# jgsimard/big-dreamer

Measured on AMD Instinct MI355X. Metric: latent transitions/sec (RSSM + imagination) at batch=50 chunk=50 H=15, higher is better.
Workload: dtype f32

## Files before the change

### big_dreamer_amd/csrc/wgrad.hip

```cpp
#include "bd_device.h"
#include "bd_host.h"
#include <stdint.h>
#include <stdlib.h>

namespace bd {

typedef float floatx16 __attribute__((ext_vector_type(16)));
constexpr int kWT = 64;
constexpr int kWM = 32;

__global__ __launch_bounds__(kThreads) void wgrad_kernel(const float* __restrict__ dpre, int ldp,
                                                         const float* __restrict__ act, int lda, int M, int N, int K,
                                                         int has_bias, int rows_per_split, float* __restrict__ ws) {
    __shared__ float P[kWM][kWT];
    __shared__ float A[kWM][kWT];
    const int Kext = K + has_bias;
    const int n0 = blockIdx.x * kWT, k0 = blockIdx.y * kWT;
    const int m_begin = blockIdx.z * rows_per_split;
    const int m_end = min(M, m_begin + rows_per_split);
    const int lane = threadIdx.x & 63, wave = threadIdx.x >> 6;
    const int wn = (wave >> 1) * 32, wk = (wave & 1) * 32;
    floatx16 acc;
#pragma unroll
    for (int i = 0; i < 16; ++i) acc[i] = 0.f;
    const int c = threadIdx.x & 63, r0 = threadIdx.x >> 6;
    for (int m0 = m_begin; m0 < m_end; m0 += kWM) {
        float pv[kWM / 4], av[kWM / 4];
#pragma unroll
        for (int i = 0; i < kWM / 4; ++i) {
            const int m = m0 + r0 + 4 * i;
            const bool ok = m < m_end;
            pv[i] = (ok && n0 + c < N) ? dpre[(size_t)m * ldp + n0 + c] : 0.f;
            const int k = k0 + c;
            av[i] = ok ? (k < K ? act[(size_t)m * lda + k] : (k == K && has_bias ? 1.f : 0.f)) : 0.f;
        }
        __syncthreads();
#pragma unroll
        for (int i = 0; i < kWM / 4; ++i) {
            P[r0 + 4 * i][c] = pv[i];
            A[r0 + 4 * i][c] = av[i];
        }
        __syncthreads();
#pragma unroll
        for (int s = 0; s < kWM / 2; ++s) {
            const float a = P[2 * s + (lane >> 5)][wn + (lane & 31)];
            const float b = A[2 * s + (lane >> 5)][wk + (lane & 31)];
            acc = __builtin_amdgcn_mfma_f32_32x32x2f32(a, b, acc, 0, 0, 0);
        }
    }
    float* slab = ws + (size_t)blockIdx.z * N * Kext;
    const int k = k0 + wk + (lane & 31);
#pragma unroll
    for (int reg = 0; reg < 16; ++reg) {
        const int n = n0 + wn + (reg & 3) + 8 * (reg >> 2) + 4 * (lane >> 5);
        if (n < N && k < Kext) slab[(size_t)n * Kext + k] = acc[reg];
    }
}

__global__ __launch_bounds__(256) void wgrad_reduce_kernel(const float* __restrict__ ws, int splits, int N, int K,
                                                           int has_bias, float* __restrict__ dW, int ldw,
                                                           float* __restrict__ db, int accumulate) {
    const int Kext = K + has_bias;
    const int total = N * Kext;
    for (int e = blockIdx.x * blockDim.x + threadIdx.x; e < total; e += gridDim.x * blockDim.x) {
        float s = 0.f;
        for (int z = 0; z < splits; ++z) s += ws[(size_t)z * total + e];
        const int n = e / Kext, k = e - n * Kext;
        float* dst = k < K ? dW + (size_t)n * ldw + k : db + n;
        *dst = accumulate ? *dst + s : s;
    }
}

__global__ __launch_bounds__(kThreads) void wgrad_grouped_kernel(const bd_wgrad_desc* __restrict__ descs, int n,
                                                                 float* __restrict__ ws) {
    __shared__ float P[kWM][kWT];
    __shared__ float A[kWM][kWT];
    int g = 0;
    while (g + 1 < n && (int)blockIdx.x >= descs[g + 1].block_begin) ++g;
    const bd_wgrad_desc d = descs[g];
    const int hb = d.db != nullptr;
    const int Kext = d.K + hb;
    int local = blockIdx.x - d.block_begin;
    const int z = local / (d.tiles_n * d.tiles_k);
    local -= z * d.tiles_n * d.tiles_k;
    const int n0 = (local / d.tiles_k) * kWT, k0 = (local % d.tiles_k) * kWT;
    const int m_begin = z * d.rows_per;
    const int m_end = min(d.M, m_begin + d.rows_per);
    const int lane = threadIdx.x & 63, wave = threadIdx.x >> 6;
    const int wn = (wave >> 1) * 32, wk = (wave & 1) * 32;
    floatx16 acc;
#pragma unroll
    for (int i = 0; i < 16; ++i) acc[i] = 0.f;
    const int c = threadIdx.x & 63, r0 = threadIdx.x >> 6;
    float pv[kWM / 4], av[kWM / 4];
    auto fetch = [&](int m0) {
#pragma unroll
        for (int i = 0; i < kWM / 4; ++i) {
            const int m = m0 + r0 + 4 * i;
            const bool ok = m < m_end;
            pv[i] = (ok && n0 + c < d.N) ? d.dpre[(size_t)m * d.ldp + n0 + c] : 0.f;
            const int k = k0 + c;
            float v = 0.f;
            if (ok) {
                if (k < d.K) v = m < d.M1 ? d.act1[(size_t)m * d.lda1 + k] : d.act2[(size_t)(m - d.M1) * d.lda2 + k];
                else if (k == d.K && hb) v = 1.f;
            }
            av[i] = v;
        }
    };
    fetch(m_begin);
    for (int m0 = m_begin; m0 < m_end; m0 += kWM) {
        __syncthreads();
#pragma unroll
        for (int i = 0; i < kWM / 4; ++i) {
            P[r0 + 4 * i][c] = pv[i];
            A[r0 + 4 * i][c] = av[i];
        }
        __syncthreads();
        if (m0 + kWM < m_end) fetch(m0 + kWM);
#pragma unroll
        for (int s = 0; s < kWM / 2; ++s) {
            const float a = P[2 * s + (lane >> 5)][wn + (lane & 31)];
            const float b = A[2 * s + (lane >> 5)][wk + (lane & 31)];
            acc = __builtin_amdgcn_mfma_f32_32x32x2f32(a, b, acc, 0, 0, 0);
        }
    }
    float* slab = ws + d.ws_off + (size_t)z * d.N * Kext;
    const int k = k0 + wk + (lane & 31);
#pragma unroll
    for (int reg = 0; reg < 16; ++reg) {
        const int nn = n0 + wn + (reg & 3) + 8 * (reg >> 2) + 4 * (lane >> 5);
        if (nn < d.N && k < Kext) slab[(size_t)nn * Kext + k] = acc[reg];
    }
}

constexpr int kWB = 13;
constexpr int kWBK = 12;
constexpr int kWBKDeep = 36;
__host__ __device__ __forceinline__ int wgrad_tiles_k(int NB, int KB, bool deep_ok) {
    if (KB <= kWB) return 1;
    return (NB <= 4 && deep_ok) ? cdiv(KB, kWBKDeep) : cdiv(KB, kWBK);
}
__host__ inline bool wgrad_act16(const bd_wgrad_desc& d) {
    auto al16 = [](const void* q) { return (reinterpret_cast<uintptr_t>(q) & 15) == 0; };
    if ((d.K & 3) != 0 || !al16(d.act1)) return false;
    if (d.g_nseg > 0) return (d.g_C & 3) == 0 && (d.g_seglen & 3) == 0;
    return (d.lda1 & 3) == 0 && (d.M1 == d.M || ((d.lda2 & 3) == 0 && al16(d.act2)));
}
constexpr int kWLd = 240;
constexpr int kWRows = 16;
constexpr int kWStage = 2 * kWRows * kWLd;
constexpr int kWRing = 3;
constexpr int kWRowsTall = 32;
constexpr int kWLdNarrow = 80;
constexpr int kWLdMid = 144;
constexpr int kWLdDeep = 592;
constexpr size_t kWideLdsBytes = 147456;
static_assert((size_t)kWRing * kWRows * (kWLdNarrow + kWLdDeep) * sizeof(float) <= kWideLdsBytes, "deep stage ring");
static_assert((size_t)kWRing * kWRowsTall * (kWLdMid + kWLd) * sizeof(float) <= kWideLdsBytes, "mid stage ring");
constexpr int kWThreads = 512;

template <int WN, int WK, int ROWS = kWRows, int PLD = kWLd, int ALD = kWLd>
__device__ __forceinline__ void wgrad_wide_body(const bd_wgrad_desc& d, float* __restrict__ ws, float* wlds, int hb, int Kext,
                                                int z, int n0, int k0, int nb_cnt, int kb_cnt) {
    const int m_begin = z * d.rows_per;
    const int m_end = min(d.M, m_begin + d.rows_per);
    const int lane = threadIdx.x & 63;
    const int wave = __builtin_amdgcn_readfirstlane(threadIdx.x >> 6);
    const int wr = wave & 1, wc = wave >> 1;
    const int hn = (nb_cnt + 1) >> 1;
    const int my_nb0 = wr ? hn : 0, my_nb = wr ? nb_cnt - hn : hn;
    const int kq = kb_cnt >> 2, krem = kb_cnt & 3;
    const int my_kb0 = wc * kq + min(wc, krem), my_kb = kq + (wc < krem ? 1 : 0);

    constexpr int kStage = ROWS * (PLD + ALD);
    constexpr int kRpw = ROWS / 8;
    static_assert(kWRing * kStage * sizeof(float) <= kWideLdsBytes, "stage ring exceeds the LDS request");
    floatx4 acc[WN][WK];
#pragma unroll
    for (int i = 0; i < WN; ++i)
#pragma unroll
        for (int j = 0; j < WK; ++j) acc[i][j] = floatx4{0.f, 0.f, 0.f, 0.f};

    typedef __attribute__((address_space(3))) void* lds_ptr_t;
    typedef const __attribute__((address_space(1))) void* glb_ptr_t;
    const int ncol = min(nb_cnt * 16, d.N - n0), kcol = min(kb_cnt * 16, d.K - k0);
    for (int i = threadIdx.x; i < kWRing * kStage; i += kWThreads) wlds[i] = 0.f;
    __syncthreads();
    if (hb && d.K >= k0 && d.K < k0 + kb_cnt * 16 && threadIdx.x < kWRing * ROWS)
        wlds[(threadIdx.x / ROWS) * kStage + ROWS * PLD + (threadIdx.x % ROWS) * ALD + (d.K - k0)] = 1.f;
    auto al16 = [](const void* q) { return (reinterpret_cast<uintptr_t>(q) & 15) == 0; };
    const bool p4 = (ncol & 3) == 0 && (d.ldp & 3) == 0 && al16(d.dpre + n0);
    const bool gathered = d.g_nseg > 0;
    const bool a4 = (kcol & 3) == 0 && (k0 & 3) == 0 &&
                    (gathered ? ((d.g_C & 3) == 0 && (d.g_seglen & 3) == 0 && al16(d.act1))
                              : ((d.lda1 & 3) == 0 && al16(d.act1) && (d.M1 == d.M || ((d.lda2 & 3) == 0 && al16(d.act2)))));
    constexpr int kCh4 = (ALD + 255) / 256;
    constexpr int kCh1 = (ALD + 63) / 64;
    constexpr int kGo = kCh1;
    int goff[kGo];
#pragma unroll
    for (int cc = 0; cc < kGo; ++cc) goff[cc] = 0;
    if (gathered) {
#pragma unroll
        for (int cc = 0; cc < kGo; ++cc) {
            const int k = k0 + (a4 ? 4 * lane + 256 * cc : lane + 64 * cc), sgm = k / d.g_seglen;
            goff[cc] = sgm * d.g_IW * d.g_C + (k - sgm * d.g_seglen);
        }
    }
    auto issue = [&](float* buf, int m0) {
#pragma unroll
        for (int rr = 0; rr < kRpw; ++rr) {
            const int m = m0 + wave * kRpw + rr;
            float* P = buf + (wave * kRpw + rr) * PLD;
            float* A = buf + ROWS * PLD + (wave * kRpw + rr) * ALD;
            if (m < m_end) {
                const float* prow = d.dpre + (size_t)m * d.ldp + n0;
                if (p4) {
                    if (4 * lane < ncol) __builtin_amdgcn_global_load_lds((glb_ptr_t)(prow + 4 * lane), (lds_ptr_t)P, 16, 0, 0);
                } else {
#pragma unroll
                    for (int cc = 0; cc < 4; ++cc) {
                        const int c = lane + 64 * cc;
                        if (c < ncol) __builtin_amdgcn_global_load_lds((glb_ptr_t)(prow + c), (lds_ptr_t)(P + 64 * cc), 4, 0, 0);
                    }
                }
                const float* abase;
                if (gathered) {
                    const int img = m / (d.g_gh * d.g_gw), rem = m - img * d.g_gh * d.g_gw;
                    const int y = rem / d.g_gw, x = rem - y * d.g_gw;
                    abase = d.act1 + (((size_t)img * d.g_IH + 2 * y) * d.g_IW + 2 * x) * d.g_C;
                } else {
                    abase = (m < d.M1 ? d.act1 + (size_t)m * d.lda1 : d.act2 + (size_t)(m - d.M1) * d.lda2) + k0;
                }
                if (a4) {
#pragma unroll
                    for (int cc = 0; cc < kCh4; ++cc)
                        if (4 * lane + 256 * cc < kcol)
                            __builtin_amdgcn_global_load_lds((glb_ptr_t)(abase + (gathered ? goff[cc] : 4 * lane + 256 * cc)),
                                                             (lds_ptr_t)(A + 256 * cc), 16, 0, 0);
                } else {
#pragma unroll
                    for (int cc = 0; cc < kCh1; ++cc) {
                        const int c = lane + 64 * cc;
                        if (c < kcol)
                            __builtin_amdgcn_global_load_lds((glb_ptr_t)(abase + (gathered ? goff[cc] : c)), (lds_ptr_t)(A + 64 * cc), 4,
                                                             0, 0);
                    }
                }
            } else {
#pragma unroll
                for (int cc = 0; cc < kCh1; ++cc) {
                    const int c = lane + 64 * cc;
                    if (c < PLD) P[c] = 0.f;
                    if (c < ALD) A[c] = 0.f;
                }
            }
        }
    };
    const int nst = cdiv(m_end - m_begin, ROWS);
    const int n_dma = kRpw * ((p4 ? 1 : cdiv(ncol, 64)) + (a4 ? cdiv(kcol, 256) : cdiv(kcol, 64)));
    auto wait_keep_newest = [&]() {
        switch (n_dma) {
            case 4: asm volatile("s_waitcnt vmcnt(4)" ::: "memory"); break;
            case 6: asm volatile("s_waitcnt vmcnt(6)" ::: "memory"); break;
            case 8: asm volatile("s_waitcnt vmcnt(8)" ::: "memory"); break;
            case 10: asm volatile("s_waitcnt vmcnt(10)" ::: "memory"); break;
            case 12: asm volatile("s_waitcnt vmcnt(12)" ::: "memory"); break;
            case 14: asm volatile("s_waitcnt vmcnt(14)" ::: "memory"); break;
            default: asm volatile("s_waitcnt vmcnt(16)" ::: "memory"); break;
        }
    };
    __syncthreads();
    issue(wlds, m_begin);
    if (nst > 1) issue(wlds + kStage, m_begin + ROWS);
    __builtin_amdgcn_s_waitcnt(0);
    __syncthreads();
    const int lrow = lane >> 4, lcol = lane & 15;
    for (int st = 0; st < nst; ++st) {
        const float* buf = wlds + (st % kWRing) * kStage;
        const bool more = st + 2 < nst;
        [[maybe_unused]] const int sb = (st == 10 || st == 11) ? (st - 10) * 8 : -1;
        BD_DSTAMP(sb, 0);
        if (more) issue(wlds + ((st + 2) % kWRing) * kStage, m_begin + (st + 2) * ROWS);
        BD_DSTAMP(sb, 1);
        const float* Pb = buf + lrow * PLD + my_nb0 * 16 + lcol;
        const float* Ab = buf + ROWS * PLD + lrow * ALD + my_kb0 * 16 + lcol;
#pragma unroll
        for (int sl = 0; sl < ROWS / 4; ++sl) {
            float a[WN], b[WK];
#pragma unroll
            for (int i = 0; i < WN; ++i) a[i] = Pb[sl * 4 * PLD + i * 16];
#pragma unroll
            for (int j = 0; j < WK; ++j) b[j] = Ab[sl * 4 * ALD + j * 16];
#pragma unroll
            for (int i = 0; i < WN; ++i)
#pragma unroll
                for (int j = 0; j < WK; ++j) acc[i][j] = mfma16(a[i], b[j], acc[i][j]);
        }
        BD_DSTAMP(sb, 2);
        if (more && st + 3 < nst) wait_keep_newest();
        else asm volatile("s_waitcnt vmcnt(0)" ::: "memory");
        BD_DSTAMP(sb, 3);
        lds_barrier();
        BD_DSTAMP(sb, 4);
    }
    float* slab = ws + d.ws_off + (size_t)z * d.N * Kext;
#pragma unroll
    for (int i = 0; i < WN; ++i) {
        if (i < my_nb) {
#pragma unroll
            for (int j = 0; j < WK; ++j) {
                if (j < my_kb) {
                    const int k = k0 + (my_kb0 + j) * 16 + lcol;
#pragma unroll
                    for (int r = 0; r < 4; ++r) {
                        const int nn = n0 + (my_nb0 + i) * 16 + 4 * lrow + r;
                        if (nn < d.N && k < Kext) slab[(size_t)nn * Kext + k] = acc[i][j][r];
                    }
                }
            }
        }
    }
}

template <int WN, int WK>
__device__ __forceinline__ void wgrad_dense_body(const bd_wgrad_desc& d, float* __restrict__ ws, float* wlds, int hb, int Kext,
                                                 int z, int n0, int k0, int nb_cnt, int kb_cnt, int my_nb0, int my_kb0) {
    const int m_begin = z * d.rows_per;
    const int m_end = min(d.M, m_begin + d.rows_per);
    const int lane = threadIdx.x & 63;
    const int wave = __builtin_amdgcn_readfirstlane(threadIdx.x >> 6);
    floatx4 acc[WN][WK];
#pragma unroll
    for (int i = 0; i < WN; ++i)
#pragma unroll
        for (int j = 0; j < WK; ++j) acc[i][j] = floatx4{0.f, 0.f, 0.f, 0.f};
    typedef __attribute__((address_space(3))) void* lds_ptr_t;
    typedef const __attribute__((address_space(1))) void* glb_ptr_t;
    const int ncol = min(nb_cnt * 16, d.N - n0), kcol = min(kb_cnt * 16, d.K - k0);
    for (int i = threadIdx.x; i < kWRing * kWStage; i += kWThreads) wlds[i] = 0.f;
    __syncthreads();
    if (hb && d.K >= k0 && d.K < k0 + kb_cnt * 16 && threadIdx.x < kWRing * kWRows)
        wlds[(threadIdx.x >> 4) * kWStage + kWRows * kWLd + (threadIdx.x & 15) * kWLd + (d.K - k0)] = 1.f;
    const bool lp = 4 * lane < ncol, la = 4 * lane < kcol;
    const float* __restrict__ pl = d.dpre + n0 + 4 * lane;
    const float* __restrict__ a1l = d.act1 + k0 + 4 * lane;
    const float* __restrict__ a2l = (d.M1 < d.M ? d.act2 : d.act1) + k0 + 4 * lane;
    auto issue = [&](float* buf, int m0) {
#pragma unroll
        for (int rr = 0; rr < 2; ++rr) {
            const int m = m0 + wave * 2 + rr;
            float* P = buf + (wave * 2 + rr) * kWLd;
            float* A = P + kWRows * kWLd;
            if (m < m_end) {
                if (lp) __builtin_amdgcn_global_load_lds((glb_ptr_t)(pl + (size_t)m * d.ldp), (lds_ptr_t)P, 16, 0, 0);
                const float* ar = m < d.M1 ? a1l + (size_t)m * d.lda1 : a2l + (size_t)(m - d.M1) * d.lda2;
                if (la) __builtin_amdgcn_global_load_lds((glb_ptr_t)ar, (lds_ptr_t)A, 16, 0, 0);
            } else {
#pragma unroll
                for (int cc = 0; cc < 4; ++cc) {
                    const int c = lane + 64 * cc;
                    if (c < kWLd) {
                        P[c] = 0.f;
                        A[c] = 0.f;
                    }
                }
            }
        }
    };
    const int nst = cdiv(m_end - m_begin, kWRows);
    __syncthreads();
    issue(wlds, m_begin);
    if (nst > 1) issue(wlds + kWStage, m_begin + kWRows);
    __builtin_amdgcn_s_waitcnt(0);
    __syncthreads();
    const int lrow = lane >> 4, lcol = lane & 15;
    for (int st = 0; st < nst; ++st) {
        const float* buf = wlds + (st % kWRing) * kWStage;
        const bool more = st + 2 < nst;
        [[maybe_unused]] const int sb = (st == 10 || st == 11) ? (st - 10) * 8 : -1;
        BD_DSTAMP(sb, 0);
        if (more && wave < 4) issue(wlds + ((st + 2) % kWRing) * kWStage, m_begin + (st + 2) * kWRows);
        BD_DSTAMP(sb, 1);
        const float* Pb = buf + lrow * kWLd + my_nb0 * 16 + lcol;
        const float* Ab = buf + kWRows * kWLd + lrow * kWLd + my_kb0 * 16 + lcol;
#pragma unroll
        for (int sl = 0; sl < kWRows / 4; ++sl) {
            float a[WN], b[WK];
#pragma unroll
            for (int i = 0; i < WN; ++i) a[i] = Pb[sl * 4 * kWLd + i * 16];
#pragma unroll
            for (int j = 0; j < WK; ++j) b[j] = Ab[sl * 4 * kWLd + j * 16];
#pragma unroll
            for (int i = 0; i < WN; ++i)
#pragma unroll
                for (int j = 0; j < WK; ++j) acc[i][j] = mfma16(a[i], b[j], acc[i][j]);
            if (sl == 1 && more && wave >= 4) issue(wlds + ((st + 2) % kWRing) * kWStage, m_begin + (st + 2) * kWRows);
        }
        BD_DSTAMP(sb, 2);
        if (more && st + 3 < nst) asm volatile("s_waitcnt vmcnt(4)" ::: "memory");
        else asm volatile("s_waitcnt vmcnt(0)" ::: "memory");
        BD_DSTAMP(sb, 3);
        lds_barrier();
        BD_DSTAMP(sb, 4);
    }
    float* slab = ws + d.ws_off + (size_t)z * d.N * Kext;
#pragma unroll
    for (int i = 0; i < WN; ++i) {
#pragma unroll
        for (int j = 0; j < WK; ++j) {
            const int k = k0 + (my_kb0 + j) * 16 + lcol;
#pragma unroll
            for (int r = 0; r < 4; ++r) {
                const int nn = n0 + (my_nb0 + i) * 16 + 4 * lrow + r;
                if (nn < d.N && k < Kext) slab[(size_t)nn * Kext + k] = acc[i][j][r];
            }
        }
    }
}

constexpr int kThinMaxKB = 7;
constexpr int kThinDpreFloats = 1024;
__host__ __device__ inline int thin_band_floats(int k, int roww) { return (k * roww + 64 + 255) & ~255; }
__host__ inline bool wgrad_thin_ok(const bd_wgrad_desc& d) {
    auto al16 = [](const void* q) { return (reinterpret_cast<uintptr_t>(q) & 15) == 0; };
    if (d.g_nseg <= 0 || d.g_C > 4 || d.N != 32 || d.ldp != 32 || d.g_gw > 32) return false;
    if (cdiv(d.K, 16) > kThinMaxKB || d.g_seglen != d.g_nseg * d.g_C) return false;
    const int roww = d.g_IW * d.g_C;
    if ((roww & 3) != 0 || !al16(d.act1) || !al16(d.dpre)) return false;
    const size_t per_wave = 2 * (size_t)(thin_band_floats(d.g_nseg, roww) + kThinDpreFloats) * sizeof(float);
    return 8 * per_wave <= kWideLdsBytes && (size_t)8 * 2 * kThinMaxKB * 1024 <= kWideLdsBytes;
}

#ifndef BD_WGRAD_TALL_MID
#define BD_WGRAD_TALL_MID 1
#endif
__device__ __forceinline__ bool tall_mid() { return BD_WGRAD_TALL_MID != 0; }

template <int KB>
__device__ __forceinline__ void wgrad_thin_body(const bd_wgrad_desc& d, float* __restrict__ ws, float* wlds, int z) {
    typedef __attribute__((address_space(3))) void* lds_ptr_t;
    typedef const __attribute__((address_space(1))) void* glb_ptr_t;
    const int lane = threadIdx.x & 63;
    const int wave = __builtin_amdgcn_readfirstlane(threadIdx.x >> 6);
    const int hb = d.db != nullptr;
    const int Kext = d.K + hb;
    const int gh = d.g_gh, gw = d.g_gw, C = d.g_C, kk = d.g_nseg;
    const int roww = d.g_IW * C, band = kk * roww, drow = gw * 32;
    const int band_al = thin_band_floats(kk, roww);
    const int per_buf = band_al + kThinDpreFloats;
    float* mine = wlds + (size_t)wave * 2 * per_buf;
    for (int i = lane; i < 2 * per_buf; i += 64) mine[i] = 0.f;
    asm volatile("s_waitcnt lgkmcnt(0)" ::: "memory");
    const int imgs = d.M / (gh * gw), ipw = d.rows_per / (gh * gw);
    const int img0 = z * ipw, img1 = min(imgs, img0 + ipw);
    const int items = (img1 - img0) * gh;
    const int nband = cdiv(band, 256), ndrow = cdiv(drow, 256);
    auto issue = [&](int it, float* buf) {
        const int img = img0 + it / gh, y = it - (it / gh) * gh;
        const float* sb = d.act1 + ((size_t)img * d.g_IH + 2 * y) * roww;
        const float* sd = d.dpre + ((size_t)img * gh + y) * gw * 32;
        for (int ch = 0; ch < nband; ++ch)
            if (4 * lane + 256 * ch < band)
                __builtin_amdgcn_global_load_lds((glb_ptr_t)(sb + 4 * lane + 256 * ch), (lds_ptr_t)(buf + 256 * ch), 16, 0, 0);
        for (int ch = 0; ch < ndrow; ++ch)
            if (4 * lane + 256 * ch < drow)
                __builtin_amdgcn_global_load_lds((glb_ptr_t)(sd + 4 * lane + 256 * ch), (lds_ptr_t)(buf + band_al + 256 * ch), 16, 0, 0);
    };
    const int n_dma = nband + ndrow;
    auto wait_keep_newest = [&]() {
        switch (n_dma) {
            case 5: asm volatile("s_waitcnt vmcnt(5)" ::: "memory"); break;
            case 6: asm volatile("s_waitcnt vmcnt(6)" ::: "memory"); break;
            case 7: asm volatile("s_waitcnt vmcnt(7)" ::: "memory"); break;
            case 8: asm volatile("s_waitcnt vmcnt(8)" ::: "memory"); break;
            case 9: asm volatile("s_waitcnt vmcnt(9)" ::: "memory"); break;
            case 10: asm volatile("s_waitcnt vmcnt(10)" ::: "memory"); break;
            default: asm volatile("s_waitcnt vmcnt(0)" ::: "memory"); break;
        }
    };
    int boff[KB];
    bool bok[KB];
#pragma unroll
    for (int kb = 0; kb < KB; ++kb) {
        const int kidx = kb * 16 + (lane & 15);
        bok[kb] = kidx < d.K;
        const int ky = kidx / d.g_seglen;
        boff[kb] = bok[kb] ? ky * roww + (kidx - ky * d.g_seglen) : 0;
    }
    floatx4 acc[2][KB];
#pragma unroll
    for (int i = 0; i < 2; ++i)
#pragma unroll
        for (int j = 0; j < KB; ++j) acc[i][j] = floatx4{0.f, 0.f, 0.f, 0.f};
    float bsum[2] = {0.f, 0.f};
    const int q = lane >> 4, n = lane & 15;
    const int nsl = cdiv(gw, 4);
    int it = wave, b = 0;
    if (it < items) issue(it, mine);
    for (; it < items; it += 8, b ^= 1) {
        const bool more = it + 8 < items;
        if (more) {
            issue(it + 8, mine + (b ^ 1) * per_buf);
            wait_keep_newest();
        } else {
            asm volatile("s_waitcnt vmcnt(0)" ::: "memory");
        }
        const float* Bd = mine + b * per_buf;
        const float* Dp = Bd + band_al;
        for (int sl = 0; sl < nsl; ++sl) {
            const int x = 4 * sl + q;
            const float a0 = Dp[x * 32 + n], a1 = Dp[x * 32 + 16 + n];
            float bv[KB];
#pragma unroll
            for (int kb = 0; kb < KB; ++kb) bv[kb] = bok[kb] ? Bd[boff[kb] + 2 * x * C] : 0.f;
#pragma unroll
            for (int kb = 0; kb < KB; ++kb) {
                acc[0][kb] = mfma16(a0, bv[kb], acc[0][kb]);
                acc[1][kb] = mfma16(a1, bv[kb], acc[1][kb]);
            }
            bsum[0] += a0;
            bsum[1] += a1;
        }
        asm volatile("s_waitcnt lgkmcnt(0)" ::: "memory");
    }
    __syncthreads();
    floatx4* R4 = reinterpret_cast<floatx4*>(wlds);
    float* BS = wlds + (size_t)8 * 2 * KB * 256;
#pragma unroll
    for (int i = 0; i < 2; ++i) {
#pragma unroll
        for (int j = 0; j < KB; ++j) R4[((wave * 2 + i) * KB + j) * 64 + lane] = acc[i][j];
        BS[(wave * 2 + i) * 64 + lane] = bsum[i];
    }
    __syncthreads();
    float* slab = ws + d.ws_off + (size_t)z * d.N * Kext;
    for (int e = threadIdx.x; e < 2 * KB * 64; e += blockDim.x) {
        const int blk = e >> 6, l = e & 63;
        floatx4 s4 = floatx4{0.f, 0.f, 0.f, 0.f};
        for (int w = 0; w < 8; ++w) s4 += R4[(w * 2 * KB + blk) * 64 + l];
        const int i = blk / KB, j = blk - i * KB;
        const int k = j * 16 + (l & 15);
        if (k < d.K) {
#pragma unroll
            for (int r = 0; r < 4; ++r) slab[(size_t)(i * 16 + 4 * (l >> 4) + r) * Kext + k] = s4[r];
        }
    }
    if (hb && threadIdx.x < 32) {
        const int i = threadIdx.x >> 4, nn = threadIdx.x & 15;
        float t = 0.f;
        for (int w = 0; w < 8; ++w)
            for (int qq = 0; qq < 4; ++qq) t += BS[(w * 2 + i) * 64 + qq * 16 + nn];
        slab[(size_t)(i * 16 + nn) * Kext + d.K] = t;
    }
}

__global__ __launch_bounds__(kWThreads) void wgrad_wide_kernel(const bd_wgrad_desc* __restrict__ descs, int n,
                                                         float* __restrict__ ws) {
    extern __shared__ float wlds[];
    int g = 0;
    while (g + 1 < n && (int)blockIdx.x >= descs[g + 1].block_begin) ++g;
    const bd_wgrad_desc d = descs[g];
    const int hb = d.db != nullptr;
    const int Kext = d.K + hb;
    const int NB = cdiv(d.N, 16), KB = cdiv(Kext, 16);
    const int nbw = cdiv(NB, d.tiles_n), kbw = cdiv(KB, d.tiles_k);
    int local = blockIdx.x - d.block_begin;
    const int z = local / (d.tiles_n * d.tiles_k);
    local -= z * d.tiles_n * d.tiles_k;
    const int tn = local / d.tiles_k, tk = local - tn * d.tiles_k;
    const int n0 = tn * nbw * 16, k0 = tk * kbw * 16;
    const int nb_cnt = min(nbw, NB - tn * nbw), kb_cnt = min(kbw, KB - tk * kbw);
    if (d.g_pad == 1) {
        const int kb_t = cdiv(d.K, 16);
        if (kb_t <= 3) wgrad_thin_body<3>(d, ws, wlds, z);
        else wgrad_thin_body<kThinMaxKB>(d, ws, wlds, z);
        return;
    }
    const int hn = (nb_cnt + 1) >> 1, hk = (kb_cnt + 3) >> 2;
    {
        auto al16 = [](const void* q) { return (reinterpret_cast<uintptr_t>(q) & 15) == 0; };
        const int ncol = min(nb_cnt * 16, d.N - n0), kcol = min(kb_cnt * 16, d.K - k0);
        const bool dense = nb_cnt == 13 && kb_cnt >= 4 && d.g_nseg == 0 && (ncol & 3) == 0 && (d.ldp & 3) == 0 &&
                           al16(d.dpre + n0) && (kcol & 3) == 0 && (k0 & 3) == 0 && (d.lda1 & 3) == 0 && al16(d.act1) &&
                           (d.M1 == d.M || ((d.lda2 & 3) == 0 && al16(d.act2)));
        if (dense) {
            const int wave = __builtin_amdgcn_readfirstlane(threadIdx.x >> 6);
            const int wr = (0xB2 >> wave) & 1;
            const int c = (0x13232100 >> (4 * wave)) & 3;
            const int kq = kb_cnt >> 2, krem = kb_cnt & 3;
            const int my_nb0 = wr ? 7 : 0, my_nb = wr ? 6 : 7;
            const int my_kb0 = c * kq + min(c, krem), my_kb = kq + (c < krem ? 1 : 0);
#define BD_WD(WN, WK) wgrad_dense_body<WN, WK>(d, ws, wlds, hb, Kext, z, n0, k0, nb_cnt, kb_cnt, my_nb0, my_kb0)
#define BD_WD_ROW(WN)                 \
    do {                              \
        if (my_kb == 4) BD_WD(WN, 4); \
        else if (my_kb == 3) BD_WD(WN, 3); \
        else if (my_kb == 2) BD_WD(WN, 2); \
        else BD_WD(WN, 1);            \
    } while (0)
            if (my_nb == 7) BD_WD_ROW(7);
            else BD_WD_ROW(6);
#undef BD_WD_ROW
#undef BD_WD
            return;
        }
    }
    if (nb_cnt <= 4) {
#define BD_WN_BODY(WN, WK) wgrad_wide_body<WN, WK, kWRowsTall, kWLdNarrow>(d, ws, wlds, hb, Kext, z, n0, k0, nb_cnt, kb_cnt)
#define BD_WN_ROW(WN)                      \
    do {                                   \
        if (hk <= 1) BD_WN_BODY(WN, 1);    \
        else if (hk <= 2) BD_WN_BODY(WN, 2); \
        else if (hk <= 3) BD_WN_BODY(WN, 3); \
        else BD_WN_BODY(WN, 4);            \
    } while (0)
        if (hk > 4) {
#define BD_WDEEP(WN, WK) wgrad_wide_body<WN, WK, kWRows, kWLdNarrow, kWLdDeep>(d, ws, wlds, hb, Kext, z, n0, k0, nb_cnt, kb_cnt)
            if (hn <= 1) { if (hk <= 8) BD_WDEEP(1, 8); else BD_WDEEP(1, 9); }
            else { if (hk <= 8) BD_WDEEP(2, 8); else BD_WDEEP(2, 9); }
#undef BD_WDEEP
            return;
        }
        if (hn <= 1) BD_WN_ROW(1);
        else BD_WN_ROW(2);
#undef BD_WN_ROW
#undef BD_WN_BODY
        return;
    }
    if (nb_cnt <= 8 && tall_mid()) {
#define BD_WM_BODY(WN, WK) wgrad_wide_body<WN, WK, kWRowsTall, kWLdMid>(d, ws, wlds, hb, Kext, z, n0, k0, nb_cnt, kb_cnt)
#define BD_WM_ROW(WN)                      \
    do {                                   \
        if (hk <= 1) BD_WM_BODY(WN, 1);    \
        else if (hk <= 2) BD_WM_BODY(WN, 2); \
        else if (hk <= 3) BD_WM_BODY(WN, 3); \
        else BD_WM_BODY(WN, 4);            \
    } while (0)
        if (hn <= 2) BD_WM_ROW(2);
        else BD_WM_ROW(4);
#undef BD_WM_ROW
#undef BD_WM_BODY
        return;
    }
#define BD_WG_BODY(WN, WK) wgrad_wide_body<WN, WK>(d, ws, wlds, hb, Kext, z, n0, k0, nb_cnt, kb_cnt)
#define BD_WG_ROW(WN)                      \
    do {                                   \
        if (hk <= 1) BD_WG_BODY(WN, 1);    \
        else if (hk <= 2) BD_WG_BODY(WN, 2); \
        else if (hk <= 3) BD_WG_BODY(WN, 3); \
        else BD_WG_BODY(WN, 4);            \
    } while (0)
    if (hn <= 1) BD_WG_ROW(1);
    else if (hn <= 2) BD_WG_ROW(2);
    else if (hn <= 4) BD_WG_ROW(4);
    else BD_WG_ROW(7);
#undef BD_WG_ROW
#undef BD_WG_BODY
}

__global__ __launch_bounds__(256) void wgrad_grouped_reduce_kernel(const bd_wgrad_desc* __restrict__ descs, int n,
                                                                   const float* __restrict__ ws) {
    int g = 0;
    while (g + 1 < n && (int)blockIdx.x >= descs[g + 1].red_begin) ++g;
    const bd_wgrad_desc d = descs[g];
    const int hb = d.db != nullptr;
    const int Kext = d.K + hb;
    const int total = d.N * Kext;
    const int e = (blockIdx.x - d.red_begin) * blockDim.x + threadIdx.x;
    if (e >= total) return;
    const float* p = ws + d.ws_off + e;
    float s = 0.f;
    for (int z = 0; z < d.splits; ++z) s += p[(size_t)z * total];
    const int nn = e / Kext, k = e - nn * Kext;
    if (k < d.K) d.dW[(size_t)nn * d.ldw + k] = s;
    else d.db[nn] = s;
}

#ifdef BD_STAMPS
extern "C" int bd_debug_wstamps(unsigned long long* out64) {
    return hipMemcpyFromSymbol(out64, HIP_SYMBOL(g_dstamps), sizeof(unsigned long long) * 64) == hipSuccess ? 0 : -1;
}
#endif

static bool wgrad_wide() {
    static const char* e = getenv("BD_WGRAD_WIDE");
    return !(e && e[0] == '0');
}
static bool thin_on() {
    static const char* e = getenv("BD_WGRAD_THIN");
    return !(e && e[0] == '0');
}
static int wgrad_rows() {
    static const char* e = getenv("BD_WGRAD_ROWS");
    const int r = e ? atoi(e) : 0;
    return r >= kWRows ? cdiv(r, kWRows) * kWRows : 0;
}

static void wgrad_plan(int M, int N, int K, int has_bias, int* splits, int* rows_per) {
    const int tiles = cdiv(N, kWT) * cdiv(K + has_bias, kWT);
    int s = 1024 / tiles;
    const int max_s = cdiv(M, 2 * kWM);
    if (s > max_s) s = max_s;
    if (s < 1) s = 1;
    int rp = cdiv(cdiv(M, s), kWM) * kWM;
    *rows_per = rp;
    *splits = cdiv(M, rp);
}

}

extern "C" {

int bd_wgrad_plan(bd_wgrad_desc* descs, int n, int* total_blocks, int* total_red_blocks, size_t* ws_floats) {
    using namespace bd;
    BD_REQUIRE(descs && n > 0 && total_blocks && total_red_blocks && ws_floats, "bd_wgrad_plan: bad arguments");
    int blocks = 0, red = 0;
    size_t off = 0;
    int rows_wide = wgrad_rows();
    if (wgrad_wide() && rows_wide == 0) {
        auto wgs = [&](int R) {
            long t = 0;
            for (int i = 0; i < n; ++i)
                t += (long)cdiv(cdiv(descs[i].N, 16), kWB) * wgrad_tiles_k(cdiv(descs[i].N, 16), cdiv(descs[i].K + (descs[i].db != nullptr), 16), wgrad_act16(descs[i])) *
                     cdiv(descs[i].M > 0 ? descs[i].M : 1, R);
            return t;
        };
        rows_wide = 128;
        while (wgs(rows_wide) > 256 && rows_wide < (1 << 20)) rows_wide += kWRows;
    }
    bool any_gather = false;
    for (int i = 0; i < n; ++i) any_gather = any_gather || descs[i].g_nseg > 0;
    auto tile_cost = [](int nb, int kb) {
        const int hn = (nb + 1) >> 1, kq = kb >> 2, kr = kb & 3;
        const int c = hn * ((kq + (0 < kr ? 1 : 0)) + (kq + (2 < kr ? 1 : 0)));
        return (c > 0 ? c : 1) + 12;
    };
    auto desc_geo = [&](const bd_wgrad_desc& d, int* tiles, int* cost) {
        const int NB = cdiv(d.N, 16), KB = cdiv(d.K + (d.db != nullptr), 16);
        const int tn = cdiv(NB, kWB), tk = wgrad_tiles_k(NB, KB, wgrad_act16(d));
        *tiles = tn * tk;
        *cost = tile_cost(cdiv(NB, tn), cdiv(KB, tk));
    };
    auto thin = [&](const bd_wgrad_desc& d) { return wgrad_wide() && thin_on() && wgrad_thin_ok(d); };
    auto rows_for = [&](const bd_wgrad_desc& d, double T) {
        int t, c;
        desc_geo(d, &t, &c);
        long r = (long)(T / c);
        r = (r / kWRows) * kWRows;
        return (int)(r < 4 * kWRows ? 4 * kWRows : (r > (1 << 22) ? (1 << 22) : r));
    };
    auto blocks_for = [&](double T) {
        long b = 0;
        for (int i = 0; i < n; ++i) {
            const bd_wgrad_desc& d = descs[i];
            if (thin(d)) {
                const int imgs = d.M / (d.g_gh * d.g_gw);
                b += cdiv(imgs, cdiv(imgs, 256));
                continue;
            }
            int t, c;
            desc_geo(d, &t, &c);
            b += (long)t * cdiv(d.M > 0 ? d.M : 1, rows_for(d, T));
        }
        return b;
    };
    double budget = 0.0;
    if (wgrad_wide() && any_gather) {
        double W = 0.0;
        for (int i = 0; i < n; ++i) {
            int t, c;
            desc_geo(descs[i], &t, &c);
            W += (double)t * (descs[i].M > 0 ? descs[i].M : 1) * c;
        }
        double R = W / (256.0 * 1024.0 * 61.0);
        if (R < 1.0) R = 1.0;
        if (R > 24.0) R = 24.0;
        const int rounds = (int)(R + 0.999);
        budget = W / (256.0 * (double)rounds);
        long target = 256L * rounds;
        if (blocks_for(budget * 8.0) > target) target += 256;
        for (int it = 0; it < 200 && blocks_for(budget) > target; ++it) budget *= 1.02;
    }
    for (int i = 0; i < n; ++i) {
        bd_wgrad_desc& d = descs[i];
        BD_REQUIRE(d.dpre && d.act1 && d.dW && d.M > 0 && d.N > 0 && d.K > 0 && d.M1 >= 0 && d.M1 <= d.M,
                   "bd_wgrad_plan: descriptor %d is malformed", i);
        BD_REQUIRE(d.M1 == d.M || d.act2, "bd_wgrad_plan: descriptor %d needs a second activation source", i);
        BD_REQUIRE(d.ldp >= d.N && (d.g_nseg > 0 || d.lda1 >= d.K) && d.ldw >= d.K && (d.M1 == d.M || d.lda2 >= d.K),
                   "bd_wgrad_plan: descriptor %d has a leading dimension that is too small", i);
        if (d.g_nseg > 0)
            BD_REQUIRE(wgrad_wide() && d.M1 == d.M && d.g_seglen > 0 && d.g_nseg * d.g_seglen == d.K && d.g_gh > 0 &&
                           d.g_gw > 0 && d.M % (d.g_gh * d.g_gw) == 0 && d.g_C > 0 && 2 * (d.g_gh - 1) + d.g_nseg <= d.g_IH &&
                           (2 * (d.g_gw - 1)) * d.g_C + d.g_seglen <= d.g_IW * d.g_C,
                       "bd_wgrad_plan: descriptor %d has an inconsistent gather geometry", i);
        const int hb = d.db != nullptr;
        d.g_pad = 0;
        if (wgrad_wide() && wgrad_thin_ok(d) && thin_on()) {
            const int px = d.g_gh * d.g_gw, imgs = d.M / px;
            const int ipw = cdiv(imgs, 256);
            d.g_pad = 1;
            d.tiles_n = d.tiles_k = 1;
            d.rows_per = ipw * px;
            d.splits = cdiv(imgs, ipw);
        } else if (wgrad_wide()) {
            d.tiles_n = cdiv(cdiv(d.N, 16), kWB);
            d.tiles_k = wgrad_tiles_k(cdiv(d.N, 16), cdiv(d.K + hb, 16), wgrad_act16(d));
            d.rows_per = rows_wide;
            if (budget > 0.0) d.rows_per = rows_for(d, budget);
            d.splits = cdiv(d.M, d.rows_per);
        } else {
            d.tiles_n = cdiv(d.N, kWT);
            d.tiles_k = cdiv(d.K + hb, kWT);
            int s = d.M / 512;
            if (s < 1) s = 1;
            if (s > 64) s = 64;
            d.rows_per = cdiv(cdiv(d.M, s), kWM) * kWM;
            d.splits = cdiv(d.M, d.rows_per);
        }
        d.block_begin = blocks;
        d.red_begin = red;
        d.ws_off = off;
        blocks += d.tiles_n * d.tiles_k * d.splits;
        red += cdiv(d.N * (d.K + hb), 256);
        off += (size_t)d.splits * d.N * (d.K + hb);
    }
    *total_blocks = blocks;
    *total_red_blocks = red;
    *ws_floats = off;
    return 0;
}

int bd_wgrad_grouped(const bd_wgrad_desc* descs_dev, int n, int total_blocks, int total_red_blocks, float* ws,
                     void* stream) {
    return bd_wgrad_grouped_phase(descs_dev, n, total_blocks, total_red_blocks, ws, 0, stream);
}

int bd_wgrad_grouped_phase(const bd_wgrad_desc* descs_dev, int n, int total_blocks, int total_red_blocks, float* ws,
                           int phase, void* stream) {
    using namespace bd;
    BD_REQUIRE(descs_dev && ws && n > 0 && n <= 4096 && total_blocks > 0 && total_red_blocks > 0 && phase >= 0 && phase <= 2,
               "bd_wgrad_grouped: bad arguments");
    if (phase == 2) {
    } else if (wgrad_wide()) {
        static_assert(kThreads == 256, "the 64x64-tile wgrad kernels are written for four waves");
        static bool lds_ok = false;
        if (!lds_ok) {
            if (allow_big_lds(wgrad_wide_kernel)) return -1;
            lds_ok = true;
        }
        hipLaunchKernelGGL(wgrad_wide_kernel, dim3(total_blocks), dim3(kWThreads), kWideLdsBytes, (hipStream_t)stream,
                           descs_dev, n, ws);
    } else {
        hipLaunchKernelGGL(wgrad_grouped_kernel, dim3(total_blocks), dim3(kThreads), 0, (hipStream_t)stream, descs_dev, n, ws);
    }
    BD_CHECK_LAUNCH("bd_wgrad_grouped");
    if (phase == 1) return 0;
    hipLaunchKernelGGL(wgrad_grouped_reduce_kernel, dim3(total_red_blocks), dim3(256), 0, (hipStream_t)stream, descs_dev, n,
                       ws);
    BD_CHECK_LAUNCH("bd_wgrad_grouped(reduce)");
    return 0;
}

size_t bd_wgrad_ws_floats(int M, int N, int K) {
    int s0, s1, rp;
    bd::wgrad_plan(M, N, K, 0, &s0, &rp);
    bd::wgrad_plan(M, N, K, 1, &s1, &rp);
    const size_t a = (size_t)s0 * N * K, b = (size_t)s1 * N * (K + 1);
    return a > b ? a : b;
}

int bd_wgrad(const float* dpre, int ldp, const float* act, int lda, int M, int N, int K, float* dW, int ldw,
             float* db, int accumulate, float* ws, size_t ws_floats, void* stream) {
    using namespace bd;
    BD_REQUIRE(dpre && act && dW && ws && M > 0 && N > 0 && K > 0, "bd_wgrad: bad arguments");
    BD_REQUIRE(ldp >= N && lda >= K && ldw >= K, "bd_wgrad: leading dimension too small");
    const int hb = db != nullptr;
    int splits, rows_per;
    wgrad_plan(M, N, K, hb, &splits, &rows_per);
    BD_REQUIRE((size_t)splits * N * (K + hb) <= ws_floats, "bd_wgrad: workspace too small (%zu floats, need %zu)",
               ws_floats, (size_t)splits * N * (K + hb));
    hipLaunchKernelGGL(wgrad_kernel, dim3(cdiv(N, kWT), cdiv(K + hb, kWT), splits), dim3(kThreads), 0,
                       (hipStream_t)stream, dpre, ldp, act, lda, M, N, K, hb, rows_per, ws);
    BD_CHECK_LAUNCH("bd_wgrad");
    const int total = N * (K + hb);
    hipLaunchKernelGGL(wgrad_reduce_kernel, dim3(cdiv(total, 256) < 1024 ? cdiv(total, 256) : 1024), dim3(256), 0,
                       (hipStream_t)stream, ws, splits, N, K, hb, dW, ldw, db, accumulate);
    BD_CHECK_LAUNCH("bd_wgrad(reduce)");
    return 0;
}

}
```

Before: 13.31 million.

## Add opt-in four-wave wgrad kernel variant and unroll split reduction

Adds a 256-thread, four-wave version of the wide weight-gradient kernel that uses a smaller LDS ring, so two workgroups can share a CU. The planner can target twice as many workgroups when this mode is selected, and the wide and dense bodies are templated on wave count with matching waitcnt depths. The new path is gated behind the BD_WGRAD_WAVES=4 environment variable, so the default path stays the eight-wave kernel. The split-K reduction kernel is also unrolled by eight to issue more loads in flight, and this part runs by default. The default in wait_keep_newest changes from vmcnt(16) to vmcnt(0), which could add stalls for unlisted DMA counts.

Measured after the change: 13.21 million, median of 3. About the same (-0.7%).

```diff
diff --git a/big_dreamer_amd/csrc/wgrad.hip b/big_dreamer_amd/csrc/wgrad.hip
--- a/big_dreamer_amd/csrc/wgrad.hip
+++ b/big_dreamer_amd/csrc/wgrad.hip
@@ -149,7 +149,6 @@
 }
 constexpr int kWLd = 240;
 constexpr int kWRows = 16;
-constexpr int kWStage = 2 * kWRows * kWLd;
 constexpr int kWRing = 3;
 constexpr int kWRowsTall = 32;
 constexpr int kWLdNarrow = 80;
@@ -160,22 +159,30 @@
 static_assert((size_t)kWRing * kWRowsTall * (kWLdMid + kWLd) * sizeof(float) <= kWideLdsBytes, "mid stage ring");
 constexpr int kWThreads = 512;
 
-template <int WN, int WK, int ROWS = kWRows, int PLD = kWLd, int ALD = kWLd>
+constexpr int kW4Threads = 256;
+constexpr int kW4Ld = 208;
+constexpr size_t kWide4LdsBytes = (size_t)kWRing * 2 * kWRows * kW4Ld * sizeof(float) + 256;
+static_assert(2 * kWide4LdsBytes <= 160 * 1024, "two 4-wave workgroups must share a CU");
+
+template <int WN, int WK, int ROWS = kWRows, int PLD = kWLd, int ALD = kWLd, int NW = 8>
 __device__ __forceinline__ void wgrad_wide_body(const bd_wgrad_desc& d, float* __restrict__ ws, float* wlds, int hb, int Kext,
                                                 int z, int n0, int k0, int nb_cnt, int kb_cnt) {
     const int m_begin = z * d.rows_per;
     const int m_end = min(d.M, m_begin + d.rows_per);
     const int lane = threadIdx.x & 63;
     const int wave = __builtin_amdgcn_readfirstlane(threadIdx.x >> 6);
+    constexpr int kCols = NW / 2;
     const int wr = wave & 1, wc = wave >> 1;
     const int hn = (nb_cnt + 1) >> 1;
     const int my_nb0 = wr ? hn : 0, my_nb = wr ? nb_cnt - hn : hn;
-    const int kq = kb_cnt >> 2, krem = kb_cnt & 3;
+    const int kq = kb_cnt / kCols, krem = kb_cnt % kCols;
     const int my_kb0 = wc * kq + min(wc, krem), my_kb = kq + (wc < krem ? 1 : 0);
 
     constexpr int kStage = ROWS * (PLD + ALD);
-    constexpr int kRpw = ROWS / 8;
-    static_assert(kWRing * kStage * sizeof(float) <= kWideLdsBytes, "stage ring exceeds the LDS request");
+    constexpr int kRpw = ROWS / NW;
+    constexpr int kNT = NW * 64;
+    static_assert(kWRing * kStage * sizeof(float) <= (NW == 8 ? kWideLdsBytes : kWide4LdsBytes),
+                  "stage ring exceeds the LDS request");
     floatx4 acc[WN][WK];
 #pragma unroll
     for (int i = 0; i < WN; ++i)
@@ -185,7 +192,7 @@
     typedef __attribute__((address_space(3))) void* lds_ptr_t;
     typedef const __attribute__((address_space(1))) void* glb_ptr_t;
     const int ncol = min(nb_cnt * 16, d.N - n0), kcol = min(kb_cnt * 16, d.K - k0);
-    for (int i = threadIdx.x; i < kWRing * kStage; i += kWThreads) wlds[i] = 0.f;
+    for (int i = threadIdx.x; i < kWRing * kStage; i += kNT) wlds[i] = 0.f;
     __syncthreads();
     if (hb && d.K >= k0 && d.K < k0 + kb_cnt * 16 && threadIdx.x < kWRing * ROWS)
         wlds[(threadIdx.x / ROWS) * kStage + ROWS * PLD + (threadIdx.x % ROWS) * ALD + (d.K - k0)] = 1.f;
@@ -268,7 +275,12 @@
             case 10: asm volatile("s_waitcnt vmcnt(10)" ::: "memory"); break;
             case 12: asm volatile("s_waitcnt vmcnt(12)" ::: "memory"); break;
             case 14: asm volatile("s_waitcnt vmcnt(14)" ::: "memory"); break;
-            default: asm volatile("s_waitcnt vmcnt(16)" ::: "memory"); break;
+            case 16: asm volatile("s_waitcnt vmcnt(16)" ::: "memory"); break;
+            case 20: asm volatile("s_waitcnt vmcnt(20)" ::: "memory"); break;
+            case 24: asm volatile("s_waitcnt vmcnt(24)" ::: "memory"); break;
+            case 28: asm volatile("s_waitcnt vmcnt(28)" ::: "memory"); break;
+            case 32: asm volatile("s_waitcnt vmcnt(32)" ::: "memory"); break;
+            default: asm volatile("s_waitcnt vmcnt(0)" ::: "memory"); break;
         }
     };
     __syncthreads();
@@ -324,13 +336,17 @@
     }
 }
 
-template <int WN, int WK>
+template <int WN, int WK, int NW = 8>
 __device__ __forceinline__ void wgrad_dense_body(const bd_wgrad_desc& d, float* __restrict__ ws, float* wlds, int hb, int Kext,
                                                  int z, int n0, int k0, int nb_cnt, int kb_cnt, int my_nb0, int my_kb0) {
     const int m_begin = z * d.rows_per;
     const int m_end = min(d.M, m_begin + d.rows_per);
     const int lane = threadIdx.x & 63;
     const int wave = __builtin_amdgcn_readfirstlane(threadIdx.x >> 6);
+    constexpr int kLd = NW == 8 ? kWLd : kW4Ld;
+    constexpr int kStage = 2 * kWRows * kLd;
+    constexpr int kRpw = kWRows / NW;
+    static_assert(kWRing * kStage * sizeof(float) <= (NW == 8 ? kWideLdsBytes : kWide4LdsBytes), "dense stage ring");
     floatx4 acc[WN][WK];
 #pragma unroll
     for (int i = 0; i < WN; ++i)
@@ -339,20 +355,20 @@
     typedef __attribute__((address_space(3))) void* lds_ptr_t;
     typedef const __attribute__((address_space(1))) void* glb_ptr_t;
     const int ncol = min(nb_cnt * 16, d.N - n0), kcol = min(kb_cnt * 16, d.K - k0);
-    for (int i = threadIdx.x; i < kWRing * kWStage; i += kWThreads) wlds[i] = 0.f;
+    for (int i = threadIdx.x; i < kWRing * kStage; i += NW * 64) wlds[i] = 0.f;
     __syncthreads();
     if (hb && d.K >= k0 && d.K < k0 + kb_cnt * 16 && threadIdx.x < kWRing * kWRows)
-        wlds[(threadIdx.x >> 4) * kWStage + kWRows * kWLd + (threadIdx.x & 15) * kWLd + (d.K - k0)] = 1.f;
+        wlds[(threadIdx.x >> 4) * kStage + kWRows * kLd + (threadIdx.x & 15) * kLd + (d.K - k0)] = 1.f;
     const bool lp = 4 * lane < ncol, la = 4 * lane < kcol;
     const float* __restrict__ pl = d.dpre + n0 + 4 * lane;
     const float* __restrict__ a1l = d.act1 + k0 + 4 * lane;
     const float* __restrict__ a2l = (d.M1 < d.M ? d.act2 : d.act1) + k0 + 4 * lane;
     auto issue = [&](float* buf, int m0) {
 #pragma unroll
-        for (int rr = 0; rr < 2; ++rr) {
-            const int m = m0 + wave * 2 + rr;
-            float* P = buf + (wave * 2 + rr) * kWLd;
-            float* A = P + kWRows * kWLd;
+        for (int rr = 0; rr < kRpw; ++rr) {
+            const int m = m0 + wave * kRpw + rr;
+            float* P = buf + (wave * kRpw + rr) * kLd;
+            float* A = P + kWRows * kLd;
             if (m < m_end) {
                 if (lp) __builtin_amdgcn_global_load_lds((glb_ptr_t)(pl + (size_t)m * d.ldp), (lds_ptr_t)P, 16, 0, 0);
                 const float* ar = m < d.M1 ? a1l + (size_t)m * d.lda1 : a2l + (size_t)(m - d.M1) * d.lda2;
@@ -361,7 +377,7 @@
 #pragma unroll
                 for (int cc = 0; cc < 4; ++cc) {
                     const int c = lane + 64 * cc;
-                    if (c < kWLd) {
+                    if (c < kLd) {
                         P[c] = 0.f;
                         A[c] = 0.f;
                     }
@@ -372,35 +388,40 @@
     const int nst = cdiv(m_end - m_begin, kWRows);
     __syncthreads();
     issue(wlds, m_begin);
-    if (nst > 1) issue(wlds + kWStage, m_begin + kWRows);
+    if (nst > 1) issue(wlds + kStage, m_begin + kWRows);
     __builtin_amdgcn_s_waitcnt(0);
     __syncthreads();
     const int lrow = lane >> 4, lcol = lane & 15;
     for (int st = 0; st < nst; ++st) {
-        const float* buf = wlds + (st % kWRing) * kWStage;
+        const float* buf = wlds + (st % kWRing) * kStage;
         const bool more = st + 2 < nst;
         [[maybe_unused]] const int sb = (st == 10 || st == 11) ? (st - 10) * 8 : -1;
         BD_DSTAMP(sb, 0);
-        if (more && wave < 4) issue(wlds + ((st + 2) % kWRing) * kWStage, m_begin + (st + 2) * kWRows);
+        if (more && (NW == 4 || wave < 4)) issue(wlds + ((st + 2) % kWRing) * kStage, m_begin + (st + 2) * kWRows);
         BD_DSTAMP(sb, 1);
-        const float* Pb = buf + lrow * kWLd + my_nb0 * 16 + lcol;
-        const float* Ab = buf + kWRows * kWLd + lrow * kWLd + my_kb0 * 16 + lcol;
+        const float* Pb = buf + lrow * kLd + my_nb0 * 16 + lcol;
+        const float* Ab = buf + kWRows * kLd + lrow * kLd + my_kb0 * 16 + lcol;
 #pragma unroll
         for (int sl = 0; sl < kWRows / 4; ++sl) {
             float a[WN], b[WK];
 #pragma unroll
-            for (int i = 0; i < WN; ++i) a[i] = Pb[sl * 4 * kWLd + i * 16];
-#pragma unroll
-            for (int j = 0; j < WK; ++j) b[j] = Ab[sl * 4 * kWLd + j * 16];
+            for (int i = 0; i < WN; ++i) a[i] = Pb[sl * 4 * kLd + i * 16];
+#pragma unroll
+            for (int j = 0; j < WK; ++j) b[j] = Ab[sl * 4 * kLd + j * 16];
 #pragma unroll
             for (int i = 0; i < WN; ++i)
 #pragma unroll
                 for (int j = 0; j < WK; ++j) acc[i][j] = mfma16(a[i], b[j], acc[i][j]);
-            if (sl == 1 && more && wave >= 4) issue(wlds + ((st + 2) % kWRing) * kWStage, m_begin + (st + 2) * kWRows);
+            if (NW == 8 && sl == 1 && more && wave >= 4)
+                issue(wlds + ((st + 2) % kWRing) * kStage, m_begin + (st + 2) * kWRows);
         }
         BD_DSTAMP(sb, 2);
-        if (more && st + 3 < nst) asm volatile("s_waitcnt vmcnt(4)" ::: "memory");
-        else asm volatile("s_waitcnt vmcnt(0)" ::: "memory");
+        if (more && st + 3 < nst) {
+            if constexpr (NW == 8) asm volatile("s_waitcnt vmcnt(4)" ::: "memory");
+            else asm volatile("s_waitcnt vmcnt(8)" ::: "memory");
+        } else {
+            asm volatile("s_waitcnt vmcnt(0)" ::: "memory");
+        }
         BD_DSTAMP(sb, 3);
         lds_barrier();
         BD_DSTAMP(sb, 4);
@@ -556,22 +577,42 @@
     }
 }
 
+struct wgrad_tile {
+    int g, z, n0, k0, nb_cnt, kb_cnt;
+};
+__device__ __forceinline__ wgrad_tile wgrad_find_tile(const bd_wgrad_desc* __restrict__ descs, int n) {
+    wgrad_tile t;
+    t.g = 0;
+    while (t.g + 1 < n && (int)blockIdx.x >= descs[t.g + 1].block_begin) ++t.g;
+    const bd_wgrad_desc& d = descs[t.g];
+    const int NB = cdiv(d.N, 16), KB = cdiv(d.K + (d.db != nullptr), 16);
+    const int nbw = cdiv(NB, d.tiles_n), kbw = cdiv(KB, d.tiles_k);
+    int local = blockIdx.x - d.block_begin;
+    t.z = local / (d.tiles_n * d.tiles_k);
+    local -= t.z * d.tiles_n * d.tiles_k;
+    const int tn = local / d.tiles_k, tk = local - tn * d.tiles_k;
+    t.n0 = tn * nbw * 16;
+    t.k0 = tk * kbw * 16;
+    t.nb_cnt = min(nbw, NB - tn * nbw);
+    t.kb_cnt = min(kbw, KB - tk * kbw);
+    return t;
+}
+__device__ __forceinline__ bool wgrad_dense_tile(const bd_wgrad_desc& d, int n0, int k0, int nb_cnt, int kb_cnt) {
+    auto al16 = [](const void* q) { return (reinterpret_cast<uintptr_t>(q) & 15) == 0; };
+    const int ncol = min(nb_cnt * 16, d.N - n0), kcol = min(kb_cnt * 16, d.K - k0);
+    return nb_cnt == 13 && kb_cnt >= 4 && d.g_nseg == 0 && (ncol & 3) == 0 && (d.ldp & 3) == 0 && al16(d.dpre + n0) &&
+           (kcol & 3) == 0 && (k0 & 3) == 0 && (d.lda1 & 3) == 0 && al16(d.act1) &&
+           (d.M1 == d.M || ((d.lda2 & 3) == 0 && al16(d.act2)));
+}
+
 __global__ __launch_bounds__(kWThreads) void wgrad_wide_kernel(const bd_wgrad_desc* __restrict__ descs, int n,
                                                          float* __restrict__ ws) {
     extern __shared__ float wlds[];
-    int g = 0;
-    while (g + 1 < n && (int)blockIdx.x >= descs[g + 1].block_begin) ++g;
-    const bd_wgrad_desc d = descs[g];
+    const wgrad_tile t = wgrad_find_tile(descs, n);
+    const bd_wgrad_desc d = descs[t.g];
     const int hb = d.db != nullptr;
     const int Kext = d.K + hb;
-    const int NB = cdiv(d.N, 16), KB = cdiv(Kext, 16);
-    const int nbw = cdiv(NB, d.tiles_n), kbw = cdiv(KB, d.tiles_k);
-    int local = blockIdx.x - d.block_begin;
-    const int z = local / (d.tiles_n * d.tiles_k);
-    local -= z * d.tiles_n * d.tiles_k;
-    const int tn = local / d.tiles_k, tk = local - tn * d.tiles_k;
-    const int n0 = tn * nbw * 16, k0 = tk * kbw * 16;
-    const int nb_cnt = min(nbw, NB - tn * nbw), kb_cnt = min(kbw, KB - tk * kbw);
+    const int z = t.z, n0 = t.n0, k0 = t.k0, nb_cnt = t.nb_cnt, kb_cnt = t.kb_cnt;
     if (d.g_pad == 1) {
         const int kb_t = cdiv(d.K, 16);
         if (kb_t <= 3) wgrad_thin_body<3>(d, ws, wlds, z);
@@ -580,12 +621,7 @@
     }
     const int hn = (nb_cnt + 1) >> 1, hk = (kb_cnt + 3) >> 2;
     {
-        auto al16 = [](const void* q) { return (reinterpret_cast<uintptr_t>(q) & 15) == 0; };
-        const int ncol = min(nb_cnt * 16, d.N - n0), kcol = min(kb_cnt * 16, d.K - k0);
-        const bool dense = nb_cnt == 13 && kb_cnt >= 4 && d.g_nseg == 0 && (ncol & 3) == 0 && (d.ldp & 3) == 0 &&
-                           al16(d.dpre + n0) && (kcol & 3) == 0 && (k0 & 3) == 0 && (d.lda1 & 3) == 0 && al16(d.act1) &&
-                           (d.M1 == d.M || ((d.lda2 & 3) == 0 && al16(d.act2)));
-        if (dense) {
+        if (wgrad_dense_tile(d, n0, k0, nb_cnt, kb_cnt)) {
             const int wave = __builtin_amdgcn_readfirstlane(threadIdx.x >> 6);
             const int wr = (0xB2 >> wave) & 1;
             const int c = (0x13232100 >> (4 * wave)) & 3;
@@ -660,6 +696,53 @@
 #undef BD_WG_BODY
 }
 
+__global__ __launch_bounds__(kW4Threads, 2) void wgrad_wide4_kernel(const bd_wgrad_desc* __restrict__ descs, int n,
+                                                                   float* __restrict__ ws) {
+    extern __shared__ float wlds[];
+    const wgrad_tile t = wgrad_find_tile(descs, n);
+    const bd_wgrad_desc d = descs[t.g];
+    const int hb = d.db != nullptr;
+    const int Kext = d.K + hb;
+    const int z = t.z, n0 = t.n0, k0 = t.k0, nb_cnt = t.nb_cnt, kb_cnt = t.kb_cnt;
+    if (wgrad_dense_tile(d, n0, k0, nb_cnt, kb_cnt)) {
+        const int wave = __builtin_amdgcn_readfirstlane(threadIdx.x >> 6);
+        const int wr = wave & 1, c = wave >> 1;
+        const int kh = (kb_cnt + 1) >> 1;
+        const int my_nb0 = wr ? 7 : 0, my_nb = wr ? 6 : 7;
+        const int my_kb0 = c ? kh : 0, my_kb = c ? kb_cnt - kh : kh;
+#define BD_WD4(WN, WK) wgrad_dense_body<WN, WK, 4>(d, ws, wlds, hb, Kext, z, n0, k0, nb_cnt, kb_cnt, my_nb0, my_kb0)
+#define BD_WD4_ROW(WN)                                 \
+    do {                                               \
+        if (my_kb == 7) BD_WD4(WN, 7);                 \
+        else if (my_kb == 6) BD_WD4(WN, 6);            \
+        else if (my_kb == 5) BD_WD4(WN, 5);            \
+        else if (my_kb == 4) BD_WD4(WN, 4);            \
+        else if (my_kb == 3) BD_WD4(WN, 3);            \
+        else BD_WD4(WN, 2);                            \
+    } while (0)
+        if (my_nb == 7) BD_WD4_ROW(7);
+        else BD_WD4_ROW(6);
+#undef BD_WD4_ROW
+#undef BD_WD4
+        return;
+    }
+    const int hn = (nb_cnt + 1) >> 1, hk = (kb_cnt + 1) >> 1;
+#define BD_WG4_BODY(WN, WK) wgrad_wide_body<WN, WK, kWRows, kW4Ld, kW4Ld, 4>(d, ws, wlds, hb, Kext, z, n0, k0, nb_cnt, kb_cnt)
+#define BD_WG4_ROW(WN)                      \
+    do {                                    \
+        if (hk <= 1) BD_WG4_BODY(WN, 1);    \
+        else if (hk <= 2) BD_WG4_BODY(WN, 2); \
+        else if (hk <= 4) BD_WG4_BODY(WN, 4); \
+        else BD_WG4_BODY(WN, 7);            \
+    } while (0)
+    if (hn <= 1) BD_WG4_ROW(1);
+    else if (hn <= 2) BD_WG4_ROW(2);
+    else if (hn <= 4) BD_WG4_ROW(4);
+    else BD_WG4_ROW(7);
+#undef BD_WG4_ROW
+#undef BD_WG4_BODY
+}
+
 __global__ __launch_bounds__(256) void wgrad_grouped_reduce_kernel(const bd_wgrad_desc* __restrict__ descs, int n,
                                                                    const float* __restrict__ ws) {
     int g = 0;
@@ -672,7 +755,15 @@
     if (e >= total) return;
     const float* p = ws + d.ws_off + e;
     float s = 0.f;
-    for (int z = 0; z < d.splits; ++z) s += p[(size_t)z * total];
+    int z = 0;
+    for (; z + 8 <= d.splits; z += 8) {
+        float v[8];
+#pragma unroll
+        for (int u = 0; u < 8; ++u) v[u] = p[(size_t)(z + u) * total];
+#pragma unroll
+        for (int u = 0; u < 8; ++u) s += v[u];
+    }
+    for (; z < d.splits; ++z) s += p[(size_t)z * total];
     const int nn = e / Kext, k = e - nn * Kext;
     if (k < d.K) d.dW[(size_t)nn * d.ldw + k] = s;
     else d.db[nn] = s;
@@ -684,6 +775,8 @@
 }
 #endif
 
+constexpr int kWRed4 = 1 << 30;
+
 static bool wgrad_wide() {
     static const char* e = getenv("BD_WGRAD_WIDE");
     return !(e && e[0] == '0');
@@ -691,6 +784,10 @@
 static bool thin_on() {
     static const char* e = getenv("BD_WGRAD_THIN");
     return !(e && e[0] == '0');
+}
+static bool waves4() {
+    static const char* e = getenv("BD_WGRAD_WAVES");
+    return e && atoi(e) == 4;
 }
 static int wgrad_rows() {
     static const char* e = getenv("BD_WGRAD_ROWS");
@@ -718,20 +815,24 @@
     BD_REQUIRE(descs && n > 0 && total_blocks && total_red_blocks && ws_floats, "bd_wgrad_plan: bad arguments");
     int blocks = 0, red = 0;
     size_t off = 0;
+    bool any_gather = false;
+    for (int i = 0; i < n; ++i) any_gather = any_gather || descs[i].g_nseg > 0;
+    const bool four = wgrad_wide() && !any_gather && waves4();
+    auto tiles_k_of = [&](const bd_wgrad_desc& d) {
+        return wgrad_tiles_k(cdiv(d.N, 16), cdiv(d.K + (d.db != nullptr), 16), !four && wgrad_act16(d));
+    };
     int rows_wide = wgrad_rows();
     if (wgrad_wide() && rows_wide == 0) {
         auto wgs = [&](int R) {
             long t = 0;
             for (int i = 0; i < n; ++i)
-                t += (long)cdiv(cdiv(descs[i].N, 16), kWB) * wgrad_tiles_k(cdiv(descs[i].N, 16), cdiv(descs[i].K + (descs[i].db != nullptr), 16), wgrad_act16(descs[i])) *
-                     cdiv(descs[i].M > 0 ? descs[i].M : 1, R);
+                t += (long)cdiv(cdiv(descs[i].N, 16), kWB) * tiles_k_of(descs[i]) * cdiv(descs[i].M > 0 ? descs[i].M : 1, R);
             return t;
         };
+        const long round = four ? 512 : 256;
         rows_wide = 128;
-        while (wgs(rows_wide) > 256 && rows_wide < (1 << 20)) rows_wide += kWRows;
-    }
-    bool any_gather = false;
-    for (int i = 0; i < n; ++i) any_gather = any_gather || descs[i].g_nseg > 0;
+        while (wgs(rows_wide) > round && rows_wide < (1 << 20)) rows_wide += kWRows;
+    }
     auto tile_cost = [](int nb, int kb) {
         const int hn = (nb + 1) >> 1, kq = kb >> 2, kr = kb & 3;
         const int c = hn * ((kq + (0 < kr ? 1 : 0)) + (kq + (2 < kr ? 1 : 0)));
@@ -806,7 +907,7 @@
             d.splits = cdiv(imgs, ipw);
         } else if (wgrad_wide()) {
             d.tiles_n = cdiv(cdiv(d.N, 16), kWB);
-            d.tiles_k = wgrad_tiles_k(cdiv(d.N, 16), cdiv(d.K + hb, 16), wgrad_act16(d));
+            d.tiles_k = tiles_k_of(d);
             d.rows_per = rows_wide;
             if (budget > 0.0) d.rows_per = rows_for(d, budget);
             d.splits = cdiv(d.M, d.rows_per);
@@ -827,7 +928,7 @@
         off += (size_t)d.splits * d.N * (d.K + hb);
     }
     *total_blocks = blocks;
-    *total_red_blocks = red;
+    *total_red_blocks = red | (four ? kWRed4 : 0);
     *ws_floats = off;
     return 0;
 }
@@ -842,7 +943,17 @@
     using namespace bd;
     BD_REQUIRE(descs_dev && ws && n > 0 && n <= 4096 && total_blocks > 0 && total_red_blocks > 0 && phase >= 0 && phase <= 2,
                "bd_wgrad_grouped: bad arguments");
+    const bool four = (total_red_blocks & kWRed4) != 0;
+    total_red_blocks &= ~kWRed4;
     if (phase == 2) {
+    } else if (four) {
+        static bool lds4_ok = false;
+        if (!lds4_ok) {
+            if (allow_big_lds(wgrad_wide4_kernel)) return -1;
+            lds4_ok = true;
+        }
+        hipLaunchKernelGGL(wgrad_wide4_kernel, dim3(total_blocks), dim3(kW4Threads), kWide4LdsBytes, (hipStream_t)stream,
+                           descs_dev, n, ws);
     } else if (wgrad_wide()) {
         static_assert(kThreads == 256, "the 64x64-tile wgrad kernels are written for four waves");
         static bool lds_ok = false;
```
